# OnurBasci/TransformerBasedNavierStokeSolver

Hardware: AMD Instinct MI355X
Metric: ns64_train_samples_per_s (higher is better)
Workload: dtype f32

## Files before the change

### transformerbasednavierstokesolver_amd/csrc/pa2d_gemm.hip

```cpp
#include "pa2d_gemm_common.h"
#include <string.h>


static Pa2dEnv read_env() {
    auto is = [](const char* n, const char* pre) { const char* e = getenv(n); return e && strncmp(e, pre, strlen(pre)) == 0; };
    auto num = [](const char* n, int dflt) { const char* e = getenv(n); return (e && e[0]) ? atoi(e) : dflt; };
    Pa2dEnv v;
    v.conv_halo = is("PA2D_CONV_HALO", "o") ? 0 : (is("PA2D_CONV_HALO", "f") ? 2 : 1);
    v.mc_big_off = is("PA2D_MC_BIG", "o") ? 1 : 0;
    v.kc_bk16 = num("PA2D_KC_BK", 0) == 16 ? 1 : 0;
    v.mc_bk = num("PA2D_MC_BK", 16) == 32 ? 32 : 16;
    v.mc_splits = num("PA2D_MC_SPLITS", 0);
    v.mcb_splits = num("PA2D_MCB_SPLITS", 0);
    v.lin_dw_split = is("PA2D_LIN_DW_SPLIT", "of") ? 0 : 1;
    v.lin_panel = is("PA2D_LIN_PANEL", "of") ? 0 : 1;
    v.lin_rowpanel = is("PA2D_LIN_ROWPANEL", "of") ? 0 : 1;
    v.lin_small_split = is("PA2D_LIN_SMALL_SPLIT", "of") ? 0 : 1;
    v.conv_mfma16 = num("PA2D_CONV_MFMA", 16) == 32 ? 0 : 1;
    v.conv_ahead = num("PA2D_CONV_AHEAD", 1) == 0 ? 0 : 1;
    v.mc_mfma16 = num("PA2D_MC_MFMA", 16) == 32 ? 0 : 1;
    v.split_big = num("PA2D_SPLIT_BIG", 1);
    v.slice_map = is("PA2D_SLICE_MAP", "l") ? 0 : 1;
    v.default_engine = is("PA2D_GEMM", "f") ? 0 : (is("PA2D_GEMM", "b") ? 2 : 1);
    return v;
}
static Pa2dEnv g_env = read_env();
const Pa2dEnv& pa2d_env() { return g_env; }
static int kc_bk(bool im2col, int Cin) {
    if (im2col && pa2d_env().kc_bk16) return 16;
    return (!im2col || (Cin % 32) == 0) ? 32 : 16;
}
KCTile kc_tile(int M, int N, bool im2col, int Cin) {
    const int tiles_m = ceil_div(M, 128);
    const long long t128 = (long long)tiles_m * ceil_div(N, 128);
    const long long t12864 = (long long)tiles_m * ceil_div(N, 64);
    const int bk = kc_bk(im2col, Cin);
    if (N > 64 && t128 >= 384) return {128, 128, bk};
    if (t12864 >= 384 || M <= 64) return {128, 64, bk};
    return {64, 64, bk};
}
bool use_split(int engine, int N, bool im2col, int Cin) {
    const int m = engine;
    if (m == 1) return im2col && N > 64 && (Cin % 32) == 0;
    if (m == 2) return N > 64 && (!im2col || (Cin % 32) == 0);
    return false;
}

int launch_kc(const KCParams& p_in, bool im2col, hipStream_t st, hipEvent_t ev0, hipEvent_t ev1) {
    KCParams p = p_in;
    if (!engine_ok(p.engine)) return PA2D_ERR_ARG;
    if (p.M <= 0 || p.N <= 0 || p.K <= 0) return PA2D_OK;
    if (!p.bias2) p.bias_split = 0x7fffffff;
    {
        const unsigned long long ab = ((unsigned long long)(p.M - 1) * p.lda + (im2col ? p.Cin : p.K)) * 4ull;
        const unsigned long long bb = ((unsigned long long)(p.N - 1) * p.ldb + p.K) * 4ull;
        if (ab >= 0xFFFFFFF0ull || bb >= 0xFFFFFFF0ull) return PA2D_ERR_UNSUPPORTED;
        p.a_bytes = (unsigned)ab;
        p.b_bytes = (unsigned)bb;
        const unsigned long long es = p.io_bf16 ? 2ull : 4ull;
        const unsigned long long cb = ((unsigned long long)(p.M - 1) * p.ldc + p.N) * es;
        const unsigned long long rb = p.res ? ((unsigned long long)(p.M - 1) * p.ldres + p.N) * es : 0ull;
        const unsigned long long xb = p.aux ? ((unsigned long long)(p.M - 1) * p.ldaux + p.N) * es : 0ull;
        if (cb >= 0xFFFFFFF0ull || rb >= 0xFFFFFFF0ull || xb >= 0xFFFFFFF0ull) return PA2D_ERR_UNSUPPORTED;
        p.c_bytes = (unsigned)cb; p.res_bytes = (unsigned)rb; p.aux_bytes = (unsigned)xb;
    }
    if ((p.K & 3) || (p.lda & 3) || (p.ldb & 3)) return PA2D_ERR_ARG;
    if (im2col && ((p.Cin & 15) || p.K != (p.taps == 27 ? 27 : 9) * p.Cin)) return PA2D_ERR_UNSUPPORTED;
    if (im2col && (p.epi != 0 || p.res)) return PA2D_ERR_ARG;
    if (ev0 && hipEventRecord(ev0, st) != hipSuccess) return PA2D_ERR_ARG;
    int rc;
    if (!im2col && p.wimg && rowpanel_applies(p)) {
        if (p.wsrc) {
            rc = launch_pack_weight_image(p.wsrc, p.wsn, p.wsk, p.wimg, p.N, p.K, st);
// ... 228 lines not shown
```

### transformerbasednavierstokesolver_amd/csrc/pa2d_gemm_mc_planes.hip

```cpp
#include "pa2d_gemm_common.h"
#include "pa2d_bf16_split.h"

struct MCPlanesParams {
    const void* PA; int chA;
    const void* PB; int chB;
    float* slab;
    int Mi, Nj, Mk, chunks_per_split, splits, H, W, Cin;
    unsigned a_bytes, b_bytes;
    int taps;
    long long lda, ldb;
    float* colsum;
};

__device__ __forceinline__ unsigned img_off(int row, int ch) {
    return 256u * row + 16u * (ch ^ (((row & 3) << 2) | ((row >> 2) & 3)));
}

template <int NT, int KS, bool F32SRC = false, bool MF16 = false>
__global__ __launch_bounds__(256, 2) void gemm_mc_planes_kernel(const MCPlanesParams p) {
    constexpr int PIMG = 4096;
    constexpr int STAGE = 2 * NT * KS * PIMG;
    constexpr int NP = 2 * NT * KS;
    __shared__ __attribute__((aligned(16))) unsigned char smem[(MF16 ? 3 : 2) * STAGE];

    const int tid = threadIdx.x, lane = tid & 63, wave = tid >> 6;
    const int tiles_i = (p.Mi + 127) / 128, tiles_j = (p.Nj + 127) / 128;
    int tj, ti, split;
    {
        const int tiles = tiles_i * tiles_j;
        if ((p.splits & 7) == 0) {
            const int xcd = blockIdx.x & 7, slot = blockIdx.x >> 3, q = p.splits >> 3;
            split = xcd * q + slot / tiles;
            const int t = slot % tiles;
            tj = t % tiles_j;
            ti = t / tiles_j;
        } else {
            tj = blockIdx.x % tiles_j;
            ti = (blockIdx.x / tiles_j) % tiles_i;
            split = blockIdx.x / tiles;
        }
    }
    const int wm = wave >> 1, wn = wave & 1;
    const int total_chunks = (p.Mk + 15) / 16;
    const int c_begin = split * p.chunks_per_split;
    const int c_end = min(total_chunks, c_begin + p.chunks_per_split);

    const int j0 = tj * 128, tap = j0 / p.Cin, cb0 = (j0 - tap * p.Cin) >> 5, ca0 = (ti * 128) >> 5;
    const int tap_dy = tap / 3 - 1, tap_dx = tap - (tap / 3) * 3 - 1, tap_shift = tap_dy * p.W + tap_dx;
    const int HW = p.H * p.W;

    const __amdgpu_buffer_rsrc_t ra_rsrc = __builtin_amdgcn_make_buffer_rsrc(const_cast<void*>(p.PA), 0, p.a_bytes, 0x00020000);
    const __amdgpu_buffer_rsrc_t rb_rsrc = __builtin_amdgcn_make_buffer_rsrc(const_cast<void*>(p.PB), 0, p.b_bytes, 0x00020000);

    int s_row[NP];
    unsigned s_goff[NP], s_lds[NP];
    bool s_isb[NP];
#pragma unroll
    for (int s = 0; s < NP; ++s) {
        const int q = tid + 256 * s;
        const int op = q / (256 * NT * KS), r = q - op * (256 * NT * KS);
        const int row = r / (16 * NT), rr = r - row * (16 * NT);
        const int c = rr / (4 * NT), pp = rr - c * (4 * NT);
        const int plane = pp >> 2, piece = pp & 3;
        s_row[s] = row;
        s_isb[s] = op != 0;
        s_goff[s] = (unsigned)((((op ? cb0 : ca0) + c) * NT + plane) * 64 + piece * 16);
        s_lds[s] = (unsigned)(((op * NT + plane) * KS + (row >> 4)) * PIMG) + img_off(row & 15, c * 4 + piece);
    }
    u32x4 rg[F32SRC ? 4 * KS : NP];
    const int frow = tid >> 4, fc8 = tid & 15;
    const unsigned flds = img_off(frow, fc8);
    const bool fok_a = ti * 128 + fc8 * 8 < p.Mi, fok_b = tj * 128 + fc8 * 8 < p.Nj;
// ... 69 lines not shown
#pragma unroll
        for (int r = 0; r < 2; ++r) {
            const int row = 8 * (kq & 1) + 4 * r + q4;
            fa[r] = img_off(row, wm * 8 + (pq >> 1)) + 8u * (pq & 1);
            fb[r] = img_off(row, wn * 8 + (pq >> 1)) + 8u * (pq & 1);
        }
        typedef __attribute__((address_space(3))) s16x4 lds_s16x4;
#define MP16_FRAG(base_, t_, pl_)                                                                         \
    __builtin_bit_cast(bf16x8, __builtin_shufflevector(                                                   \
        __builtin_amdgcn_ds_read_tr16_b64_v4i16((lds_s16x4*)(smem + ((base_[0] ^ ((unsigned)(t_) << 5)) + (pl_) * PIMG))), \
        __builtin_amdgcn_ds_read_tr16_b64_v4i16((lds_s16x4*)(smem + ((base_[1] ^ ((unsigned)(t_) << 5)) + (pl_) * PIMG))), \
        0, 1, 2, 3, 4, 5, 6, 7))
#define MP16_MMA(ib_, AF)                                                                                 \
    _Pragma("unroll") for (int j = 0; j < 4; ++j) {        \
        acc[ib_][j] = __builtin_amdgcn_mfma_f32_16x16x32_bf16(xf[j][1], AF[1], acc[ib_][j], 0, 0, 0);     \
        acc[ib_][j] = __builtin_amdgcn_mfma_f32_16x16x32_bf16(xf[j][0], AF[2], acc[ib_][j], 0, 0, 0);     \
        acc[ib_][j] = __builtin_amdgcn_mfma_f32_16x16x32_bf16(xf[j][2], AF[0], acc[ib_][j], 0, 0, 0);     \
        acc[ib_][j] = __builtin_amdgcn_mfma_f32_16x16x32_bf16(xf[j][0], AF[1], acc[ib_][j], 0, 0, 0);     \
        acc[ib_][j] = __builtin_amdgcn_mfma_f32_16x16x32_bf16(xf[j][1], AF[0], acc[ib_][j], 0, 0, 0);     \
        acc[ib_][j] = __builtin_amdgcn_mfma_f32_16x16x32_bf16(xf[j][0], AF[0], acc[ib_][j], 0, 0, 0);     \
    }
        bf16x8 pk[2][NT];
#define MP16_CONVERT()                                                                                    \
    _Pragma("unroll") for (int op = 0; op < 2; ++op) {                                                    \
        const u32x4 u0_ = rg[op * 2], u1_ = rg[op * 2 + 1];                                               \
        const float4 v0_ = make_float4(__uint_as_float(u0_.x), __uint_as_float(u0_.y), __uint_as_float(u0_.z), __uint_as_float(u0_.w)); \
        const float4 v1_ = make_float4(__uint_as_float(u1_.x), __uint_as_float(u1_.y), __uint_as_float(u1_.z), __uint_as_float(u1_.w)); \
        if (op == 0 && do_cs) {                                                                           \
            cs[0] += v0_.x; cs[1] += v0_.y; cs[2] += v0_.z; cs[3] += v0_.w;                               \
            cs[4] += v1_.x; cs[5] += v1_.y; cs[6] += v1_.z; cs[7] += v1_.w;                               \
        }                                                                                                 \
        bf16x4 h0_, m0_, l0_, h1_, m1_, l1_;                                                              \
        split3(v0_, h0_, m0_, l0_);                                                                       \
        split3(v1_, h1_, m1_, l1_);                                                                       \
        pk[op][0] = __builtin_shufflevector(h0_, h1_, 0, 1, 2, 3, 4, 5, 6, 7);                            \
        pk[op][1] = __builtin_shufflevector(m0_, m1_, 0, 1, 2, 3, 4, 5, 6, 7);                            \
        pk[op][2] = __builtin_shufflevector(l0_, l1_, 0, 1, 2, 3, 4, 5, 6, 7);                            \
    }
#define MP16_WRITE(buf_)                                                                                  \
    _Pragma("unroll") for (int op = 0; op < 2; ++op) _Pragma("unroll") for (int pl = 0; pl < NT; ++pl)    \
        *reinterpret_cast<bf16x8*>(smem + (buf_) * STAGE + flds + (op * NT + pl) * PIMG) = pk[op][pl];
        const int nst = c_end - c_begin, steps = (nst + 1) >> 1;
        if (nst > 0) {
            MP_LOAD(c_begin)
            MP16_CONVERT()
            MP16_WRITE(0)
            MP_LOAD(c_begin + 1)
            MP16_CONVERT()
            MP16_WRITE(1)
            if (steps > 1) { MP_LOAD(c_begin + 2) }
        }
        __syncthreads();
        int sp = 0, sq = 1, sr = 2;
        for (int k = 0; k < steps; ++k) {
            const bool has_next = k + 1 < steps;
            const unsigned lo = (unsigned)((kq >> 1) ? sq : sp) * (unsigned)STAGE;
            const unsigned ua[2] = {fa[0] + lo, fa[1] + lo};
            const unsigned ub[2] = {fb[0] + lo + NT * PIMG, fb[1] + lo + NT * PIMG};
            bf16x8 xf[4][NT];
#pragma unroll
            for (int j = 0; j < 4; ++j)
#pragma unroll
                for (int pl = 0; pl < NT; ++pl) xf[j][pl] = MP16_FRAG(ub, j, pl);
            bf16x8 afc[NT], afn[NT];
#pragma unroll
            for (int pl = 0; pl < NT; ++pl) afc[pl] = MP16_FRAG(ua, 0, pl);
#pragma unroll
            for (int ib = 0; ib < 4; ++ib) {
                if (ib < 3) {
#pragma unroll
                    for (int pl = 0; pl < NT; ++pl) afn[pl] = MP16_FRAG(ua, ib + 1, pl);
                }
                if (ib == 1 && has_next) {
                    MP16_CONVERT()
                    MP16_WRITE(sr)
                    MP_LOAD(c_begin + 2 * k + 3)
                }
                if (ib == 3) {
                    if (has_next) {
                        MP16_CONVERT()
                        if (k + 2 < steps) { MP_LOAD(c_begin + 2 * k + 4) }
                    }
                    __syncthreads();
                    if (has_next) { MP16_WRITE(sp) }
                }
                MP16_MMA(ib, afc)
#pragma unroll
                for (int pl = 0; pl < NT; ++pl) afc[pl] = afn[pl];
            }
            __syncthreads();
            const int t = sp;
            sp = sr;
            sr = sq;
            sq = t;
        }
#undef MP16_CONVERT
#undef MP16_WRITE
#undef MP16_MMA
#undef MP16_FRAG
        if (do_cs) {
            float* sm = reinterpret_cast<float*>(smem);
#pragma unroll
            for (int e = 0; e < 8; ++e) sm[frow * 128 + fc8 * 8 + e] = cs[e];
            __syncthreads();
            if (tid < 128) {
                float t = 0.f;
// ... 58 lines not shown
                const s16x4 b0 = __builtin_amdgcn_ds_read_tr16_b64_v4i16((lds_s16x4*)(st + (NT + pl) * KS * PIMG + fb[t][0]));
                const s16x4 b1 = __builtin_amdgcn_ds_read_tr16_b64_v4i16((lds_s16x4*)(st + (NT + pl) * KS * PIMG + fb[t][1]));
                const s16x8 av = __builtin_shufflevector(a0, a1, 0, 1, 2, 3, 4, 5, 6, 7);
                const s16x8 bv = __builtin_shufflevector(b0, b1, 0, 1, 2, 3, 4, 5, 6, 7);
                af[t][pl] = __builtin_bit_cast(bf16x8, av);
                bf[t][pl] = __builtin_bit_cast(bf16x8, bv);
            }
#pragma unroll
        for (int i = 0; i < 2; ++i)
#pragma unroll
            for (int j = 0; j < 2; ++j) {
                if constexpr (NT == 3) {
                    acc[i][j] = __builtin_amdgcn_mfma_f32_32x32x16_bf16(af[i][1], bf[j][1], acc[i][j], 0, 0, 0);
                    acc[i][j] = __builtin_amdgcn_mfma_f32_32x32x16_bf16(af[i][2], bf[j][0], acc[i][j], 0, 0, 0);
                    acc[i][j] = __builtin_amdgcn_mfma_f32_32x32x16_bf16(af[i][0], bf[j][2], acc[i][j], 0, 0, 0);
                    acc[i][j] = __builtin_amdgcn_mfma_f32_32x32x16_bf16(af[i][1], bf[j][0], acc[i][j], 0, 0, 0);
                    acc[i][j] = __builtin_amdgcn_mfma_f32_32x32x16_bf16(af[i][0], bf[j][1], acc[i][j], 0, 0, 0);
                }
                acc[i][j] = __builtin_amdgcn_mfma_f32_32x32x16_bf16(af[i][0], bf[j][0], acc[i][j], 0, 0, 0);
            }
        }
        if (c + KS < c_end) { MP_STORE(buf ^ 1) }
        __syncthreads();
    }
#undef MP_LOAD
#undef MP_STORE

    if constexpr (F32SRC) {
        if (do_cs) {
            float* sm = reinterpret_cast<float*>(smem);
#pragma unroll
            for (int e = 0; e < 8; ++e) sm[frow * 128 + fc8 * 8 + e] = cs[e];
            __syncthreads();
            if (tid < 128) {
                float t = 0.f;
#pragma unroll
                for (int r = 0; r < 16; ++r) t += sm[r * 128 + tid];
                if (ti * 128 + tid < p.Mi) p.colsum[(size_t)split * p.Mi + ti * 128 + tid] = t;
            }
        }
    }
    float* out = p.slab + (size_t)split * p.Mi * p.Nj;
    const int col0 = tj * 128 + wn * 64 + (lane & 31);
    const int row0 = ti * 128 + wm * 64 + 4 * (lane >> 5);
#pragma unroll
    for (int j = 0; j < 2; ++j)
#pragma unroll
        for (int i = 0; i < 2; ++i)
#pragma unroll
            for (int r = 0; r < 16; ++r) {
                const int row = row0 + i * 32 + (r & 3) + 8 * (r >> 2);
                if (!F32SRC || (row < p.Mi && col0 + j * 32 < p.Nj)) out[(size_t)row * p.Nj + col0 + j * 32] = acc[i][j][r];
            }
}

bool mc_planes_supported(int C, int Cin) { return (C % 64) == 0 && (Cin % 128) == 0; }

int launch_mc_planes(const void* PA, const void* PB, int C, int Cin, int Mk, int H, int W, float* slab,
                     const MCPlan& pl, int NT, hipStream_t st) {
    if (!mc_planes_supported(C, Cin) || !pl.big) return PA2D_ERR_UNSUPPORTED;
    MCPlanesParams p;
    p.PA = PA; p.chA = 2 * C / 32; p.PB = PB; p.chB = Cin / 32; p.slab = slab;
    p.Mi = 2 * C; p.Nj = 9 * Cin; p.Mk = Mk; p.chunks_per_split = pl.chunks_per_split; p.splits = pl.splits;
    p.H = H; p.W = W; p.Cin = Cin; p.taps = 9;
    const unsigned long long ab = (unsigned long long)Mk * p.chA * NT * 64, bb = (unsigned long long)Mk * p.chB * NT * 64;
    if (ab >= 0xFFFFFFF0ull || bb >= 0xFFFFFFF0ull) return PA2D_ERR_UNSUPPORTED;
    p.a_bytes = (unsigned)ab; p.b_bytes = (unsigned)bb;
    const dim3 grid((p.Mi / 128) * (p.Nj / 128) * pl.splits);
    if (NT == 3) hipLaunchKernelGGL((gemm_mc_planes_kernel<3, 1>), grid, dim3(256), 0, st, p);
    else hipLaunchKernelGGL((gemm_mc_planes_kernel<1, 4>), grid, dim3(256), 0, st, p);
    PA2D_CHECK_LAUNCH();
    return PA2D_OK;
}

template <int NT, int KS, bool MF16 = false>
__global__ __launch_bounds__(512, 1) void gemm_mc_planes_big_kernel(const MCPlanesParams p, const int per_xcd) {
    constexpr int PIMG = 8192;
    constexpr int STAGE = 2 * NT * KS * PIMG;
    constexpr int NP = (2 * NT * KS * 512) / 512;
    extern __shared__ __attribute__((aligned(16))) unsigned char smem[];

    const int tid = threadIdx.x, lane = tid & 63, wave = tid >> 6;
    const int tiles_i = (p.Mi + 255) / 256, tiles_j = (p.Nj + 255) / 256;
    const int tiles = tiles_i * tiles_j;
    const int lin = (blockIdx.x & 7) * per_xcd + (blockIdx.x >> 3);
    if ((int)(blockIdx.x >> 3) >= per_xcd || lin >= tiles * p.splits) return;
    const int split = lin / tiles, t_ = lin - split * tiles;
    const int ti = t_ / tiles_j, tj = t_ - ti * tiles_j;
    const int wm = wave >> 2, wn = wave & 3;
    const int total_chunks = (p.Mk + 15) / 16;
    const int c_begin = split * p.chunks_per_split;
    const int c_end = min(total_chunks, c_begin + p.chunks_per_split);
    const int HW = p.taps == 1 ? 1 : p.H * p.W;

    const __amdgpu_buffer_rsrc_t ra_rsrc = __builtin_amdgcn_make_buffer_rsrc(const_cast<void*>(p.PA), 0, p.a_bytes, 0x00020000);
    const __amdgpu_buffer_rsrc_t rb_rsrc = __builtin_amdgcn_make_buffer_rsrc(const_cast<void*>(p.PB), 0, p.b_bytes, 0x00020000);

    const int row16 = tid >> 5, cgrp = (tid & 31) >> 2, piece = tid & 3;
    const bool colok_a = ti * 256 + cgrp * 32 < p.Mi;
    const unsigned goff_a = (unsigned)((((ti * 256) >> 5) + cgrp) * NT * 64 + piece * 16);
    const int jc = tj * 256 + cgrp * 32;
    const int tap = p.taps == 1 ? 4 : jc / p.Cin;
    const bool colok_b = jc < p.Nj;
    const unsigned goff_b = (unsigned)((p.taps == 1 ? (jc >> 5) : ((jc - tap * p.Cin) >> 5)) * NT * 64 + piece * 16);
    const int tap_dy = tap / 3 - 1, tap_dx = tap - (tap / 3) * 3 - 1, tap_shift = tap_dy * p.W + tap_dx;
    const unsigned pitch_a = (unsigned)(p.chA * NT * 64), pitch_b = (unsigned)(p.chB * NT * 64);
    const unsigned lds_off = 512u * row16 + 16u * ((unsigned)(cgrp * 4 + piece) ^ (unsigned)(((row16 & 3) << 2) | ((row16 >> 2) & 3)));
#define MB_LOAD(c_, RG)                                                                                   \
    {                                                                                                     \
        _Pragma("unroll") for (int ks = 0; ks < KS; ++ks) {                                               \
            const int m_ = ((c_) + ks) * 16 + row16;                                                      \
            const bool okr_ = m_ < p.Mk && (c_) + ks < c_end;             \
            bool okb_ = okr_ && colok_b;                                                                  \
            int mm_ = m_;                                                                                 \
            if (p.taps != 1) {       \
                okb_ = okb_ && (unsigned)(ly + tap_dy) < (unsigned)p.H && (unsigned)(lx + tap_dx) < (unsigned)p.W; \
                mm_ = m_ + tap_shift;                                                                     \
                lx += 16;                                                                                 \
                while (lx >= p.W) { lx -= p.W; ++ly; }                                                    \
                while (ly >= p.H) ly -= p.H;                                                              \
            }                                                                                             \
            const unsigned oa_ = (okr_ && colok_a) ? (unsigned)m_ * pitch_a + goff_a : OOB_OFF;           \
            const unsigned ob_ = okb_ ? (unsigned)mm_ * pitch_b + goff_b : OOB_OFF;                       \
            _Pragma("unroll") for (int pl = 0; pl < NT; ++pl) {                                           \
                RG[pl * KS + ks] = __builtin_amdgcn_raw_buffer_load_b128(ra_rsrc, oa_ == OOB_OFF ? OOB_OFF : oa_ + pl * 64u, 0, 0); \
                RG[(NT + pl) * KS + ks] = __builtin_amdgcn_raw_buffer_load_b128(rb_rsrc, ob_ == OOB_OFF ? OOB_OFF : ob_ + pl * 64u, 0, 0); \
            }                                                                                             \
        }                                                                                                 \
    }
// ... 1 lines not shown
    {                                                                                                     \
        _Pragma("unroll") for (int s = 0; s < NP; ++s)                                                    \
            *reinterpret_cast<u32x4*>(smem + (buf_) * STAGE + s * PIMG + lds_off) = RG[s];                \
    }
    u32x4 rg0[NP];
    int ly = 0, lx = 0;
    if (p.taps != 1) {
        const int n0 = (c_begin * 16 + row16) % HW;
        ly = n0 / p.W;
        lx = n0 - ly * p.W;
    }

    if constexpr (MF16) {
        static_assert(NT == 3 && KS == 1, "the 16x16x32 form is written for the split engine");
        f32x4 acc[8][4];
#pragma unroll
        for (int i = 0; i < 8; ++i)
#pragma unroll
            for (int j = 0; j < 4; ++j) acc[i][j] = f32x4{0.f, 0.f, 0.f, 0.f};
        const int kq = lane >> 4, q4 = (lane & 15) >> 2, pq = lane & 3;
        unsigned fa[2], fb[2];
#pragma unroll
        for (int r = 0; r < 2; ++r) {
            const int row = 8 * (kq & 1) + 4 * r + q4;
            const unsigned swz = (unsigned)(((row & 3) << 2) | ((row >> 2) & 3));
            fa[r] = 512u * row + 16u * ((unsigned)(wm * 16 + (pq >> 1)) ^ swz) + 8u * (pq & 1);
            fb[r] = 512u * row + 16u * ((unsigned)(wn * 8 + (pq >> 1)) ^ swz) + 8u * (pq & 1);
        }
        typedef __attribute__((address_space(3))) s16x4 lds_s16x4;
#define MB16_FRAG(base_, t_, pl_)                                                                         \
    __builtin_bit_cast(bf16x8, __builtin_shufflevector(                                                   \
        __builtin_amdgcn_ds_read_tr16_b64_v4i16((lds_s16x4*)(smem + ((base_[0] ^ ((unsigned)(t_) << 5)) + (pl_) * PIMG))), \
        __builtin_amdgcn_ds_read_tr16_b64_v4i16((lds_s16x4*)(smem + ((base_[1] ^ ((unsigned)(t_) << 5)) + (pl_) * PIMG))), \
        0, 1, 2, 3, 4, 5, 6, 7))
#define MB16_MMA(ib_, AF)                                                                                 \
    _Pragma("unroll") for (int j = 0; j < 4; ++j) {        \
        acc[ib_][j] = __builtin_amdgcn_mfma_f32_16x16x32_bf16(xf[j][1], AF[1], acc[ib_][j], 0, 0, 0);     \
        acc[ib_][j] = __builtin_amdgcn_mfma_f32_16x16x32_bf16(xf[j][0], AF[2], acc[ib_][j], 0, 0, 0);     \
        acc[ib_][j] = __builtin_amdgcn_mfma_f32_16x16x32_bf16(xf[j][2], AF[0], acc[ib_][j], 0, 0, 0);     \
        acc[ib_][j] = __builtin_amdgcn_mfma_f32_16x16x32_bf16(xf[j][0], AF[1], acc[ib_][j], 0, 0, 0);     \
        acc[ib_][j] = __builtin_amdgcn_mfma_f32_16x16x32_bf16(xf[j][1], AF[0], acc[ib_][j], 0, 0, 0);     \
        acc[ib_][j] = __builtin_amdgcn_mfma_f32_16x16x32_bf16(xf[j][0], AF[0], acc[ib_][j], 0, 0, 0);     \
    }
        const int nst = c_end - c_begin, steps = (nst + 1) >> 1;
        if (nst > 0) {
            MB_LOAD(c_begin, rg0)
            MB_STORE(0, rg0)
            MB_LOAD(c_begin + 1, rg0)
            MB_STORE(1, rg0)
            if (steps > 1) MB_LOAD(c_begin + 2, rg0)
        }
        __syncthreads();
        int sp = 0, sq = 1, sr = 2;
        for (int k = 0; k < steps; ++k) {
            const unsigned lo = (unsigned)((kq >> 1) ? sq : sp) * (unsigned)STAGE;
            const unsigned ua[2] = {fa[0] + lo, fa[1] + lo};
            const unsigned ub[2] = {fb[0] + lo + NT * PIMG, fb[1] + lo + NT * PIMG};
            bf16x8 xf[4][NT];
#pragma unroll
            for (int j = 0; j < 4; ++j)
#pragma unroll
                for (int pl = 0; pl < NT; ++pl) xf[j][pl] = MB16_FRAG(ub, j, pl);
            bf16x8 afc[NT], afn[NT];
#pragma unroll
            for (int pl = 0; pl < NT; ++pl) afc[pl] = MB16_FRAG(ua, 0, pl);
#pragma unroll
            for (int ib = 0; ib < 8; ++ib) {
                if (ib < 7) {
#pragma unroll
                    for (int pl = 0; pl < NT; ++pl) afn[pl] = MB16_FRAG(ua, ib + 1, pl);
                }
                if (ib == 4) {
                    MB_STORE(sr, rg0)
                    MB_LOAD(c_begin + 2 * k + 3, rg0)
                }
                if (ib == 7) {
                    __syncthreads();
                    MB_STORE(sp, rg0)
                    MB_LOAD(c_begin + 2 * k + 4, rg0)
                }
                MB16_MMA(ib, afc)
#pragma unroll
                for (int pl = 0; pl < NT; ++pl) afc[pl] = afn[pl];
            }
            __syncthreads();
            const int t = sp;
            sp = sr;
            sr = sq;
            sq = t;
        }
#undef MB16_MMA
#undef MB16_FRAG
        float* out = p.slab + (size_t)split * p.Mi * p.Nj;
#pragma unroll
        for (int j = 0; j < 4; ++j) {
            const int col = tj * 256 + wn * 64 + j * 16 + 4 * kq;
            if (col >= p.Nj) continue;
#pragma unroll
            for (int ib = 0; ib < 8; ++ib) {
                const int row = ti * 256 + wm * 128 + ib * 16 + (lane & 15);
                if (row < p.Mi) *reinterpret_cast<f32x4*>(out + (size_t)row * p.Nj + col) = acc[ib][j];
            }
        }
        return;
    }

// ... 38 lines not shown
                const s16x4 b0 = __builtin_amdgcn_ds_read_tr16_b64_v4i16((lds_s16x4*)(st + (NT + pl) * KS * PIMG + fb[t][0])); \
                const s16x4 b1 = __builtin_amdgcn_ds_read_tr16_b64_v4i16((lds_s16x4*)(st + (NT + pl) * KS * PIMG + fb[t][1])); \
                bf[t][pl] = __builtin_bit_cast(bf16x8, __builtin_shufflevector(b0, b1, 0, 1, 2, 3, 4, 5, 6, 7)); \
            }                                                                                             \
        }                                                                                                 \
        _Pragma("unroll") for (int i = 0; i < 4; ++i)                                                     \
            _Pragma("unroll") for (int j = 0; j < 2; ++j) {                                               \
                if constexpr (NT == 3) {                                        \
                    acc[i][j] = __builtin_amdgcn_mfma_f32_32x32x16_bf16(af[i][1], bf[j][1], acc[i][j], 0, 0, 0); \
                    acc[i][j] = __builtin_amdgcn_mfma_f32_32x32x16_bf16(af[i][2], bf[j][0], acc[i][j], 0, 0, 0); \
                    acc[i][j] = __builtin_amdgcn_mfma_f32_32x32x16_bf16(af[i][0], bf[j][2], acc[i][j], 0, 0, 0); \
                    acc[i][j] = __builtin_amdgcn_mfma_f32_32x32x16_bf16(af[i][1], bf[j][0], acc[i][j], 0, 0, 0); \
                    acc[i][j] = __builtin_amdgcn_mfma_f32_32x32x16_bf16(af[i][0], bf[j][1], acc[i][j], 0, 0, 0); \
                }                                                                                         \
                acc[i][j] = __builtin_amdgcn_mfma_f32_32x32x16_bf16(af[i][0], bf[j][0], acc[i][j], 0, 0, 0); \
            }                                                                                             \
    }
    if (c_begin < c_end) {
        MB_LOAD(c_begin, rg0)
        MB_STORE(0, rg0)
        if (c_begin + KS < c_end) MB_LOAD(c_begin + KS, rg0)
    }
    __syncthreads();
    for (int c = c_begin; c < c_end; c += KS) {
        const int buf = ((c - c_begin) / KS) & 1;
        if (c + KS < c_end) {
            MB_STORE(buf ^ 1, rg0)
            if (c + 2 * KS < c_end) MB_LOAD(c + 2 * KS, rg0)
        }
        MB_COMPUTE(buf)
        __syncthreads();
    }
#undef MB_COMPUTE
#undef MB_LOAD
#undef MB_STORE

    float* out = p.slab + (size_t)split * p.Mi * p.Nj;
    const int col0 = tj * 256 + wn * 64 + (lane & 31);
    const int row0 = ti * 256 + wm * 128 + 4 * (lane >> 5);
#pragma unroll
    for (int j = 0; j < 2; ++j) {
        const int col = col0 + j * 32;
        if (col >= p.Nj) continue;
#pragma unroll
        for (int i = 0; i < 4; ++i)
#pragma unroll
            for (int r = 0; r < 16; ++r) {
                const int row = row0 + i * 32 + (r & 3) + 8 * (r >> 2);
                if (row < p.Mi) out[(size_t)row * p.Nj + col] = acc[i][j][r];
            }
    }
}

MCPlan plan_mc_planes_big(int Mi, int Nj, int Mk) {
    MCPlan pl;
    if (Mk < 1) Mk = 1;
    pl.big = 2;
    const int tiles = ceil_div(Mi, 256) * ceil_div(Nj, 256);
    const int total_chunks = ceil_div(Mk, 16);
    int splits = 256 / tiles;
    if (pa2d_env().mcb_splits > 0) splits = pa2d_env().mcb_splits;
    const int max_splits = total_chunks / 8 > 0 ? total_chunks / 8 : 1;
    if (splits > max_splits) splits = max_splits;
    if (splits < 1) splits = 1;
    pl.chunks_per_split = ceil_div(total_chunks, splits);
    pl.splits = ceil_div(total_chunks, pl.chunks_per_split);
    pl.slab_floats = (size_t)pl.splits * Mi * Nj;
    return pl;
}

bool mc_planes_big_applies(int C, int Cin, int Mk) {
    if (pa2d_env().mc_big_off) return false;
    return (C % 16) == 0 && (Cin % 32) == 0 && 2 * C >= 256 && 9 * Cin >= 256 && Mk >= 16 * 8 * 4;
}

int launch_mc_planes_big(const void* PA, const void* PB, int C, int Cin, int Mk, int H, int W, float* slab,
                         const MCPlan& pl, int NT, hipStream_t st) {
    return launch_mc_planes_big_raw(PA, 2 * C, PB, Cin, 9, Mk, H, W, slab, pl, NT, st);
}

int launch_mc_planes_big_raw(const void* PA, int Mi, const void* PB, int Cin, int taps, int Mk, int H, int W, float* slab,
                             const MCPlan& pl, int NT, hipStream_t st) {
    if ((Mi & 31) || (Cin & 31) || (taps != 1 && taps != 9)) return PA2D_ERR_UNSUPPORTED;
    MCPlanesParams p;
    p.PA = PA; p.chA = Mi / 32; p.PB = PB; p.chB = Cin / 32; p.slab = slab;
    p.Mi = Mi; p.Nj = taps * Cin; p.Mk = Mk; p.chunks_per_split = pl.chunks_per_split; p.splits = pl.splits;
    p.H = H; p.W = W; p.Cin = Cin; p.taps = taps;
    const unsigned long long ab = (unsigned long long)Mk * p.chA * NT * 64, bb = (unsigned long long)Mk * p.chB * NT * 64;
    if (ab >= 0xFFFFFFF0ull || bb >= 0xFFFFFFF0ull) return PA2D_ERR_UNSUPPORTED;
    p.a_bytes = (unsigned)ab; p.b_bytes = (unsigned)bb;
    const int wgs = ceil_div(p.Mi, 256) * ceil_div(p.Nj, 256) * pl.splits;
    const int per_xcd = ceil_div(wgs, 8);
    const dim3 grid(per_xcd * 8);
    if (NT == 3 && pa2d_env().mc_mfma16 && (reinterpret_cast<uintptr_t>(slab) & 15) == 0) {
        const int smem = 3 * 2 * 3 * 1 * 8192;
        {
            hipError_t e = hipFuncSetAttribute(reinterpret_cast<const void*>(&gemm_mc_planes_big_kernel<3, 1, true>),
                                               hipFuncAttributeMaxDynamicSharedMemorySize, smem);
            if (e != hipSuccess) return (int)e;
        }
        hipLaunchKernelGGL((gemm_mc_planes_big_kernel<3, 1, true>), grid, dim3(512), smem, st, p, per_xcd);
    } else if (NT == 3) {
        const int smem = 2 * 2 * 3 * 1 * 8192;
        {
            hipError_t e = hipFuncSetAttribute(reinterpret_cast<const void*>(&gemm_mc_planes_big_kernel<3, 1>),
                                               hipFuncAttributeMaxDynamicSharedMemorySize, smem);
            if (e != hipSuccess) return (int)e;
        }
        hipLaunchKernelGGL((gemm_mc_planes_big_kernel<3, 1>), grid, dim3(512), smem, st, p, per_xcd);
    } else {
        const int smem = 2 * 2 * 1 * 4 * 8192;
        {
            hipError_t e = hipFuncSetAttribute(reinterpret_cast<const void*>(&gemm_mc_planes_big_kernel<1, 4>),
                                               hipFuncAttributeMaxDynamicSharedMemorySize, smem);
            if (e != hipSuccess) return (int)e;
        }
        hipLaunchKernelGGL((gemm_mc_planes_big_kernel<1, 4>), grid, dim3(512), smem, st, p, per_xcd);
    }
    PA2D_CHECK_LAUNCH();
    return PA2D_OK;
}

bool mc_f32src_applies(int Mi, int Nj, int Mk, long long lda, long long ldb) {
    return pa2d_env().lin_dw_split && (Mi % 8) == 0 && (Nj % 8) == 0 && Mi > 64 && Nj > 64 && Mk >= 16 * 8 * 16 && (lda % 4) == 0 && (ldb % 4) == 0;
}

int launch_mc_f32src(const float* A, long long lda, int Mi, const float* B, long long ldb, int Nj, int Mk, float* slab,
                     const MCPlan& pl, int NT, float* colsum, hipStream_t st) {
    if (!pl.big) return PA2D_ERR_UNSUPPORTED;
    MCPlanesParams p = {};
    p.PA = A; p.PB = B; p.slab = slab; p.lda = lda; p.ldb = ldb; p.colsum = colsum;
    p.Mi = Mi; p.Nj = Nj; p.Mk = Mk; p.chunks_per_split = pl.chunks_per_split; p.splits = pl.splits;
    p.H = 1; p.W = 1; p.Cin = Nj; p.taps = 1; p.chA = 0; p.chB = 0;
    const unsigned long long ab = ((unsigned long long)(Mk - 1) * lda + Mi) * 4ull, bb = ((unsigned long long)(Mk - 1) * ldb + Nj) * 4ull;
    if (ab >= 0xFFFFFFF0ull || bb >= 0xFFFFFFF0ull) return PA2D_ERR_UNSUPPORTED;
    p.a_bytes = (unsigned)ab; p.b_bytes = (unsigned)bb;
    const dim3 grid(ceil_div(Mi, 128) * ceil_div(Nj, 128) * pl.splits);
    if (NT == 3 && pa2d_env().mc_mfma16 && (Nj % 4) == 0 && (reinterpret_cast<uintptr_t>(slab) & 15) == 0)
        hipLaunchKernelGGL((gemm_mc_planes_kernel<3, 1, true, true>), grid, dim3(256), 0, st, p);
    else if (NT == 3) hipLaunchKernelGGL((gemm_mc_planes_kernel<3, 1, true>), grid, dim3(256), 0, st, p);
    else hipLaunchKernelGGL((gemm_mc_planes_kernel<1, 4, true>), grid, dim3(256), 0, st, p);
    PA2D_CHECK_LAUNCH();
    return PA2D_OK;
}
```

### transformerbasednavierstokesolver_amd/csrc/pa2d_internal.h

```cpp
#pragma once
#include <hip/hip_runtime.h>
#include <stdint.h>

typedef float f32x16 __attribute__((ext_vector_type(16)));
typedef float f32x4 __attribute__((ext_vector_type(4)));

#define PA2D_OK 0
#define PA2D_ERR_ARG 1001
#define PA2D_ERR_UNSUPPORTED 1002
#define PA2D_ERR_WORKSPACE 1003

#define PA2D_CHECK_LAUNCH()                         \
    do {                                            \
        hipError_t e__ = hipGetLastError();         \
        if (e__ != hipSuccess) return (int)e__;     \
    } while (0)

enum { ACT_NONE = 0, ACT_GELU = 1, ACT_TANH = 2, ACT_SIGMOID = 3, ACT_RELU = 4, ACT_SOFTPLUS = 5,
       ACT_ELU = 6, ACT_SILU = 7 };

__device__ __forceinline__ float normal_cdf(float x, float& e_out) {
#pragma clang fp contract(off)
    const float z = fabsf(x) * 0.70710678118654752440f;
    const float t = __builtin_amdgcn_rcpf(fmaf(0.3275911f, z, 1.0f));
// ... 48 lines not shown
#pragma unroll
    for (int o = 32; o > 0; o >>= 1) v += __shfl_xor(v, o, 64);
    return v;
}
__device__ __forceinline__ float wave_max(float v) {
#pragma unroll
    for (int o = 32; o > 0; o >>= 1) v = fmaxf(v, __shfl_xor(v, o, 64));
    return v;
}

typedef unsigned int u32x4 __attribute__((ext_vector_type(4)));
#define OOB_OFF 0xFFFFFFFFu

__device__ __forceinline__ __amdgpu_buffer_rsrc_t make_rsrc(const float* base, unsigned bytes) {
    return __builtin_amdgcn_make_buffer_rsrc(const_cast<float*>(base), 0, bytes, 0x00020000);
}
__device__ __forceinline__ float4 buf_load4(__amdgpu_buffer_rsrc_t r, unsigned voff) {
    const u32x4 v = __builtin_amdgcn_raw_buffer_load_b128(r, voff, 0, 0);
    return make_float4(__uint_as_float(v.x), __uint_as_float(v.y), __uint_as_float(v.z), __uint_as_float(v.w));
}


__device__ __forceinline__ float buf_load1(__amdgpu_buffer_rsrc_t r, unsigned voff) {
    return __uint_as_float(__builtin_amdgcn_raw_buffer_load_b32(r, voff, 0, 0));
}
__device__ __forceinline__ void buf_store1(__amdgpu_buffer_rsrc_t r, unsigned voff, float v) {
    __builtin_amdgcn_raw_buffer_store_b32(__float_as_uint(v), r, voff, 0, 0);
}

__device__ __forceinline__ float2 buf_load2(__amdgpu_buffer_rsrc_t r, unsigned voff) {
    typedef unsigned int u32x2_ __attribute__((ext_vector_type(2)));
    const u32x2_ v = __builtin_amdgcn_raw_buffer_load_b64(r, voff, 0, 0);
    return make_float2(__uint_as_float(v.x), __uint_as_float(v.y));
}
__device__ __forceinline__ void buf_store4(__amdgpu_buffer_rsrc_t r, unsigned voff, float4 v) {
    u32x4 u = {__float_as_uint(v.x), __float_as_uint(v.y), __float_as_uint(v.z), __float_as_uint(v.w)};
    __builtin_amdgcn_raw_buffer_store_b128(u, r, voff, 0, 0);
}

#define PA2D_ACT_SAVE_DERIVATIVE_BIT 0x100

struct Pa2dEnv {
    int conv_halo;
    int mc_big_off;
    int kc_bk16;
    int mc_bk;
    int mc_splits;
    int mcb_splits;
    int lin_dw_split;
    int lin_panel;
    int conv_mfma16;
    int conv_ahead;
    int mc_mfma16;
    int lin_small_split;
    int lin_rowpanel;
    int split_big;
    int slice_map;
    int default_engine;
};
const Pa2dEnv& pa2d_env();

static inline int pa2d_zero(void* p, size_t bytes, hipStream_t st) {
    if (!p || !bytes) return PA2D_OK;
    return (int)hipMemsetAsync(p, 0, bytes, st);
}
static inline int ceil_div(int a, int b) { return (a + b - 1) / b; }
static inline long long ceil_div_ll(long long a, long long b) { return (a + b - 1) / b; }

struct ReduceSegs { int nseg; long long begin[5]; float* dst[4]; };
int pa2d_launch_reduce_segs(const float* slab, int nslab, long long count, const ReduceSegs& segs, int accumulate,
                            hipStream_t st);

typedef __bf16 bf16_t;
template <typename T> struct Act;
template <> struct Act<float> {
    static constexpr unsigned ES = 4;
    static __device__ __forceinline__ float4 ld4(const float* p) { return *reinterpret_cast<const float4*>(p); }
    static __device__ __forceinline__ void st4(float* p, float4 v) { *reinterpret_cast<float4*>(p) = v; }
    static __device__ __forceinline__ float ld1(const float* p) { return *p; }
    static __device__ __forceinline__ float4 bld4(__amdgpu_buffer_rsrc_t r, unsigned off) { return buf_load4(r, off); }
    static __device__ __forceinline__ float2 bld2(__amdgpu_buffer_rsrc_t r, unsigned off) { return buf_load2(r, off); }
    static __device__ __forceinline__ float bld1(__amdgpu_buffer_rsrc_t r, unsigned off) { return buf_load1(r, off); }
    static __device__ __forceinline__ float bld1s(__amdgpu_buffer_rsrc_t r, unsigned off, unsigned soff) {
        return __uint_as_float(__builtin_amdgcn_raw_buffer_load_b32(r, off, soff, 0));
    }
    static __device__ __forceinline__ void bst4(__amdgpu_buffer_rsrc_t r, unsigned off, float4 v) { buf_store4(r, off, v); }
    static __device__ __forceinline__ void bst1(__amdgpu_buffer_rsrc_t r, unsigned off, float v) { buf_store1(r, off, v); }
};
__device__ __forceinline__ float bf16_bits_to_f32(unsigned short b) { return __uint_as_float((unsigned)b << 16); }
__device__ __forceinline__ unsigned short f32_to_bf16_bits(float x) {
    const bf16_t h = (bf16_t)x;
    return __builtin_bit_cast(unsigned short, h);
}
__device__ __forceinline__ unsigned pack_bf16x2(float lo, float hi) {
    return (unsigned)f32_to_bf16_bits(lo) | ((unsigned)f32_to_bf16_bits(hi) << 16);
}
template <> struct Act<bf16_t> {
    static constexpr unsigned ES = 2;
    static __device__ __forceinline__ float4 unpack4(uint2 q) {
        return make_float4(__uint_as_float(q.x << 16), __uint_as_float(q.x & 0xFFFF0000u), __uint_as_float(q.y << 16),
                           __uint_as_float(q.y & 0xFFFF0000u));
    }
    static __device__ __forceinline__ float4 ld4(const bf16_t* p) { return unpack4(*reinterpret_cast<const uint2*>(p)); }
    static __device__ __forceinline__ void st4(bf16_t* p, float4 v) {
        *reinterpret_cast<uint2*>(p) = make_uint2(pack_bf16x2(v.x, v.y), pack_bf16x2(v.z, v.w));
    }
// ... 52 lines not shown
```

Measured before the change: 73.38.

## Software-pipeline MC planes GEMM inner loop with fragment look-ahead and pinned schedule

Adds an AHEAD variant of the small and big MC-planes split-K GEMM kernels. It prefetches LDS fragments for the next block while MFMAs run, interleaves global loads, bf16 conversion and LDS stores between MFMA groups, and pins the order with sched_barrier. The aim is to hide LDS and global latency behind the MFMA work. The new path is the default, selected through PA2D_MC_AHEAD=3, and the old loop stays as reference kernels; the cost is higher register pressure and a more fragile hand-written schedule.

```diff
diff --git a/transformerbasednavierstokesolver_amd/csrc/pa2d_gemm.hip b/transformerbasednavierstokesolver_amd/csrc/pa2d_gemm.hip
--- a/transformerbasednavierstokesolver_amd/csrc/pa2d_gemm.hip
+++ b/transformerbasednavierstokesolver_amd/csrc/pa2d_gemm.hip
@@ -19,6 +19,7 @@
     v.conv_mfma16 = num("PA2D_CONV_MFMA", 16) == 32 ? 0 : 1;
     v.conv_ahead = num("PA2D_CONV_AHEAD", 1) == 0 ? 0 : 1;
     v.mc_mfma16 = num("PA2D_MC_MFMA", 16) == 32 ? 0 : 1;
+    v.mc_ahead = num("PA2D_MC_AHEAD", 3) & 3;
     v.split_big = num("PA2D_SPLIT_BIG", 1);
     v.slice_map = is("PA2D_SLICE_MAP", "l") ? 0 : 1;
     v.default_engine = is("PA2D_GEMM", "f") ? 0 : (is("PA2D_GEMM", "b") ? 2 : 1);
diff --git a/transformerbasednavierstokesolver_amd/csrc/pa2d_gemm_mc_planes.hip b/transformerbasednavierstokesolver_amd/csrc/pa2d_gemm_mc_planes.hip
--- a/transformerbasednavierstokesolver_amd/csrc/pa2d_gemm_mc_planes.hip
+++ b/transformerbasednavierstokesolver_amd/csrc/pa2d_gemm_mc_planes.hip
@@ -16,8 +16,8 @@
     return 256u * row + 16u * (ch ^ (((row & 3) << 2) | ((row >> 2) & 3)));
 }
 
-template <int NT, int KS, bool F32SRC = false, bool MF16 = false>
-__global__ __launch_bounds__(256, 2) void gemm_mc_planes_kernel(const MCPlanesParams p) {
+template <int NT, int KS, bool F32SRC, bool MF16, bool AHEAD>
+__device__ __forceinline__ void mc_planes_body(const MCPlanesParams& p) {
     constexpr int PIMG = 4096;
     constexpr int STAGE = 2 * NT * KS * PIMG;
     constexpr int NP = 2 * NT * KS;
@@ -193,6 +193,80 @@
         }
         __syncthreads();
         int sp = 0, sq = 1, sr = 2;
+        if constexpr (AHEAD) {
+            bf16x8 xf[4][NT], a0[NT], a1[NT];
+            unsigned ua[2], ub[2];
+#pragma unroll
+            for (int r = 0; r < 2; ++r) {
+                ua[r] = fa[r] + (unsigned)(kq >> 1) * (unsigned)STAGE;
+                ub[r] = fb[r] + (unsigned)(kq >> 1) * (unsigned)STAGE + NT * PIMG;
+            }
+#define MC_PIN() __builtin_amdgcn_sched_barrier(0)
+#define MC_LDA(AF_, t_)                                                                                   \
+    {                                                                                                     \
+        _Pragma("unroll") for (int pl = 0; pl < NT; ++pl) AF_[pl] = MP16_FRAG(ua, t_, pl);                \
+        MC_PIN();                                                                                         \
+    }
+#define MC_LDX(j_)                                                                                        \
+    {                                                                                                     \
+        _Pragma("unroll") for (int pl = 0; pl < NT; ++pl) xf[j_][pl] = MP16_FRAG(ub, j_, pl);             \
+        MC_PIN();                                                                                         \
+    }
+#define MC_T(ib_, j_, AF_, xq_, aq_) \
+    acc[ib_][j_] = __builtin_amdgcn_mfma_f32_16x16x32_bf16(xf[j_][xq_], AF_[aq_], acc[ib_][j_], 0, 0, 0);
+#define MC_MM(ib_, j_, AF_)                           \
+    {                                                                                                     \
+        MC_T(ib_, j_, AF_, 1, 1) MC_T(ib_, j_, AF_, 0, 2) MC_T(ib_, j_, AF_, 2, 0)                        \
+        MC_T(ib_, j_, AF_, 0, 1) MC_T(ib_, j_, AF_, 1, 0) MC_T(ib_, j_, AF_, 0, 0)                        \
+        MC_PIN();                                                                                         \
+    }
+            MC_PIN();
+            MC_LDA(a0, 0) MC_LDX(0) MC_LDX(1) MC_LDX(2)
+            for (int k = 0; k < steps; ++k) {
+                const bool has_next = k + 1 < steps;
+                MC_PIN();
+                MC_MM(0, 0, a0) MC_LDX(3)
+                MC_MM(0, 1, a0) MC_LDA(a1, 1)
+                MC_MM(0, 2, a0) MC_MM(0, 3, a0)
+                MC_LDA(a0, 2)
+                if (has_next) { MP16_CONVERT() }
+                MP16_WRITE(sr)
+                if (has_next) { MP_LOAD(c_begin + 2 * k + 3) }
+                MC_PIN();
+                MC_MM(1, 0, a1) MC_MM(1, 1, a1) MC_MM(1, 2, a1) MC_MM(1, 3, a1)
+                MC_LDA(a1, 3)
+                {
+                    const unsigned d = (unsigned)(((kq >> 1) ? sp - sq : sr - sp) * STAGE);
+#pragma unroll
+                    for (int r = 0; r < 2; ++r) { ua[r] += d; ub[r] += d; }
+                    MC_PIN();
+                }
+                MC_MM(2, 0, a0) MC_MM(2, 1, a0)
+                if (has_next) {
+                    MP16_CONVERT()
+                    if (k + 2 < steps) { MP_LOAD(c_begin + 2 * k + 4) }
+                }
+                __syncthreads();
+                MC_PIN();
+                MP16_WRITE(sp)
+                MC_PIN();
+                MC_MM(3, 0, a1) MC_MM(3, 1, a1) MC_MM(2, 2, a0) MC_MM(2, 3, a0)
+                __syncthreads();
+                MC_PIN();
+                MC_LDA(a0, 0) MC_LDX(0)
+                MC_MM(3, 2, a1) MC_LDX(1)
+                MC_MM(3, 3, a1) MC_LDX(2)
+                const int t = sp;
+                sp = sr;
+                sr = sq;
+                sq = t;
+            }
+#undef MC_MM
+#undef MC_T
+#undef MC_LDX
+#undef MC_LDA
+#undef MC_PIN
+        } else
         for (int k = 0; k < steps; ++k) {
             const bool has_next = k + 1 < steps;
             const unsigned lo = (unsigned)((kq >> 1) ? sq : sp) * (unsigned)STAGE;
@@ -357,6 +431,14 @@
                 const int row = row0 + i * 32 + (r & 3) + 8 * (r >> 2);
                 if (!F32SRC || (row < p.Mi && col0 + j * 32 < p.Nj)) out[(size_t)row * p.Nj + col0 + j * 32] = acc[i][j][r];
             }
+}
+
+template <int NT, int KS, bool F32SRC = false, bool MF16 = false>
+__global__ __launch_bounds__(256, 2) void gemm_mc_planes_kernel(const MCPlanesParams p) {
+    mc_planes_body<NT, KS, F32SRC, MF16, MF16>(p);
+}
+__global__ __launch_bounds__(256, 2) void gemm_mc_planes_ref_kernel(const MCPlanesParams p) {
+    mc_planes_body<3, 1, true, true, false>(p);
 }
 
 bool mc_planes_supported(int C, int Cin) { return (C % 64) == 0 && (Cin % 128) == 0; }
@@ -378,8 +460,8 @@
     return PA2D_OK;
 }
 
-template <int NT, int KS, bool MF16 = false>
-__global__ __launch_bounds__(512, 1) void gemm_mc_planes_big_kernel(const MCPlanesParams p, const int per_xcd) {
+template <int NT, int KS, bool MF16, bool AHEAD>
+__device__ __forceinline__ void mc_planes_big_body(const MCPlanesParams& p, const int per_xcd) {
     constexpr int PIMG = 8192;
     constexpr int STAGE = 2 * NT * KS * PIMG;
     constexpr int NP = (2 * NT * KS * 512) / 512;
@@ -487,6 +569,83 @@
         }
         __syncthreads();
         int sp = 0, sq = 1, sr = 2;
+        if constexpr (AHEAD) {
+            bf16x8 xf[4][NT], a0[NT], a1[NT];
+            unsigned ua[2], ub[2];
+#pragma unroll
+            for (int r = 0; r < 2; ++r) {
+                ua[r] = fa[r] + (unsigned)(kq >> 1) * (unsigned)STAGE;
+                ub[r] = fb[r] + (unsigned)(kq >> 1) * (unsigned)STAGE + NT * PIMG;
+            }
+#define MC_PIN() __builtin_amdgcn_sched_barrier(0)
+#define MC_LDA(AF_, t_)                                                                                   \
+    {                                                                                                     \
+        _Pragma("unroll") for (int pl = 0; pl < NT; ++pl) AF_[pl] = MB16_FRAG(ua, t_, pl);                \
+        MC_PIN();                                                                                         \
+    }
+#define MC_LDX(j_)                                                                                        \
+    {                                                                                                     \
+        _Pragma("unroll") for (int pl = 0; pl < NT; ++pl) xf[j_][pl] = MB16_FRAG(ub, j_, pl);             \
+        MC_PIN();                                                                                         \
+    }
+#define MC_T(ib_, j_, AF_, xq_, aq_) \
+    acc[ib_][j_] = __builtin_amdgcn_mfma_f32_16x16x32_bf16(xf[j_][xq_], AF_[aq_], acc[ib_][j_], 0, 0, 0);
+#define MC_MM(ib_, j_, AF_)                           \
+    {                                                                                                     \
+        MC_T(ib_, j_, AF_, 1, 1) MC_T(ib_, j_, AF_, 0, 2) MC_T(ib_, j_, AF_, 2, 0)                        \
+        MC_T(ib_, j_, AF_, 0, 1) MC_T(ib_, j_, AF_, 1, 0) MC_T(ib_, j_, AF_, 0, 0)                        \
+        MC_PIN();                                                                                         \
+    }
+#define MC_BLOCK(ib_, AF_) MC_MM(ib_, 0, AF_) MC_MM(ib_, 1, AF_) MC_MM(ib_, 2, AF_) MC_MM(ib_, 3, AF_)
+#define MC_ST(buf_, s_) *reinterpret_cast<u32x4*>(smem + (buf_) * STAGE + (s_) * PIMG + lds_off) = rg0[s_];
+            MC_PIN();
+            MC_LDA(a0, 0) MC_LDX(0) MC_LDX(1) MC_LDX(2)
+            for (int k = 0; k < steps; ++k) {
+                MC_PIN();
+                MC_MM(0, 0, a0) MC_LDX(3)
+                MC_MM(0, 1, a0) MC_LDA(a1, 1)
+                MC_MM(0, 2, a0) MC_MM(0, 3, a0)
+                MC_LDA(a0, 2) MC_BLOCK(1, a1)
+                MC_LDA(a1, 3) MC_BLOCK(2, a0)
+                MC_LDA(a0, 4) MC_BLOCK(3, a1)
+                MC_LDA(a1, 5)
+                MC_MM(4, 0, a0) MC_ST(sr, 0) MC_ST(sr, 1) MC_ST(sr, 2) MC_PIN();
+                MC_MM(4, 1, a0) MC_ST(sr, 3) MC_ST(sr, 4) MC_ST(sr, 5) MC_PIN();
+                MC_MM(4, 2, a0) MB_LOAD(c_begin + 2 * k + 3, rg0) MC_PIN();
+                MC_MM(4, 3, a0)
+                MC_LDA(a0, 6) MC_BLOCK(5, a1)
+                MC_LDA(a1, 7)
+                {
+                    const unsigned d = (unsigned)(((kq >> 1) ? sp - sq : sr - sp) * STAGE);
+#pragma unroll
+                    for (int r = 0; r < 2; ++r) { ua[r] += d; ub[r] += d; }
+                    MC_PIN();
+                }
+                MC_MM(6, 0, a0) MC_MM(6, 1, a0)
+                __syncthreads();
+                MC_PIN();
+                MB_STORE(sp, rg0)
+                MB_LOAD(c_begin + 2 * k + 4, rg0)
+                MC_PIN();
+                MC_MM(7, 0, a1) MC_MM(7, 1, a1) MC_MM(6, 2, a0) MC_MM(6, 3, a0)
+                __syncthreads();
+                MC_PIN();
+                MC_LDA(a0, 0) MC_LDX(0)
+                MC_MM(7, 2, a1) MC_LDX(1)
+                MC_MM(7, 3, a1) MC_LDX(2)
+                const int t = sp;
+                sp = sr;
+                sr = sq;
+                sq = t;
+            }
+#undef MC_ST
+#undef MC_BLOCK
+#undef MC_MM
+#undef MC_T
+#undef MC_LDX
+#undef MC_LDA
+#undef MC_PIN
+        } else
         for (int k = 0; k < steps; ++k) {
             const unsigned lo = (unsigned)((kq >> 1) ? sq : sp) * (unsigned)STAGE;
             const unsigned ua[2] = {fa[0] + lo, fa[1] + lo};
@@ -631,6 +790,14 @@
     }
 }
 
+template <int NT, int KS, bool MF16 = false>
+__global__ __launch_bounds__(512, 1) void gemm_mc_planes_big_kernel(const MCPlanesParams p, const int per_xcd) {
+    mc_planes_big_body<NT, KS, MF16, MF16>(p, per_xcd);
+}
+__global__ __launch_bounds__(512, 1) void gemm_mc_planes_big_ref_kernel(const MCPlanesParams p, const int per_xcd) {
+    mc_planes_big_body<3, 1, true, false>(p, per_xcd);
+}
+
 MCPlan plan_mc_planes_big(int Mi, int Nj, int Mk) {
     MCPlan pl;
     if (Mk < 1) Mk = 1;
@@ -673,12 +840,13 @@
     const dim3 grid(per_xcd * 8);
     if (NT == 3 && pa2d_env().mc_mfma16 && (reinterpret_cast<uintptr_t>(slab) & 15) == 0) {
         const int smem = 3 * 2 * 3 * 1 * 8192;
+        auto* const kern = (pa2d_env().mc_ahead & 1) ? &gemm_mc_planes_big_kernel<3, 1, true> : &gemm_mc_planes_big_ref_kernel;
         {
-            hipError_t e = hipFuncSetAttribute(reinterpret_cast<const void*>(&gemm_mc_planes_big_kernel<3, 1, true>),
+            hipError_t e = hipFuncSetAttribute(reinterpret_cast<const void*>(kern),
                                                hipFuncAttributeMaxDynamicSharedMemorySize, smem);
             if (e != hipSuccess) return (int)e;
         }
-        hipLaunchKernelGGL((gemm_mc_planes_big_kernel<3, 1, true>), grid, dim3(512), smem, st, p, per_xcd);
+        hipLaunchKernelGGL(kern, grid, dim3(512), smem, st, p, per_xcd);
     } else if (NT == 3) {
         const int smem = 2 * 2 * 3 * 1 * 8192;
         {
@@ -715,9 +883,10 @@
     if (ab >= 0xFFFFFFF0ull || bb >= 0xFFFFFFF0ull) return PA2D_ERR_UNSUPPORTED;
     p.a_bytes = (unsigned)ab; p.b_bytes = (unsigned)bb;
     const dim3 grid(ceil_div(Mi, 128) * ceil_div(Nj, 128) * pl.splits);
-    if (NT == 3 && pa2d_env().mc_mfma16 && (Nj % 4) == 0 && (reinterpret_cast<uintptr_t>(slab) & 15) == 0)
-        hipLaunchKernelGGL((gemm_mc_planes_kernel<3, 1, true, true>), grid, dim3(256), 0, st, p);
-    else if (NT == 3) hipLaunchKernelGGL((gemm_mc_planes_kernel<3, 1, true>), grid, dim3(256), 0, st, p);
+    if (NT == 3 && pa2d_env().mc_mfma16 && (Nj % 4) == 0 && (reinterpret_cast<uintptr_t>(slab) & 15) == 0) {
+        if (pa2d_env().mc_ahead & 2) hipLaunchKernelGGL((gemm_mc_planes_kernel<3, 1, true, true>), grid, dim3(256), 0, st, p);
+        else hipLaunchKernelGGL(gemm_mc_planes_ref_kernel, grid, dim3(256), 0, st, p);
+    } else if (NT == 3) hipLaunchKernelGGL((gemm_mc_planes_kernel<3, 1, true>), grid, dim3(256), 0, st, p);
     else hipLaunchKernelGGL((gemm_mc_planes_kernel<1, 4, true>), grid, dim3(256), 0, st, p);
     PA2D_CHECK_LAUNCH();
     return PA2D_OK;
diff --git a/transformerbasednavierstokesolver_amd/csrc/pa2d_internal.h b/transformerbasednavierstokesolver_amd/csrc/pa2d_internal.h
--- a/transformerbasednavierstokesolver_amd/csrc/pa2d_internal.h
+++ b/transformerbasednavierstokesolver_amd/csrc/pa2d_internal.h
@@ -124,6 +124,7 @@
     int conv_mfma16;
     int conv_ahead;
     int mc_mfma16;
+    int mc_ahead;
     int lin_small_split;
     int lin_rowpanel;
     int split_big;
```

New measurement: 73.69, median of 6. No clear change (+0.4%).
